# ai-forever/Kandinsky-2

Measured on AMD Instinct MI355X. Metric: UNet denoise steps/sec @ 768x768 bs=1, 50 steps, higher is better.
Workload: dtype bf16; 1 GPU; Kandinsky-2.x text2img 768x768, decoder_steps=50, bs=1/GPU (CFG batch 2x4x96x96), 2.1-architecture UNet (1.23B) p_sampler step; parity pinned against the reference's modules; head=2.1, tile_configs_measured_in_this_process=0, images_per_gpu=1, parallelism=prompt-sharded x1, weights by one RCCL broadcast, world_size_observed=1, graph=True, chains=1, loop_graph=a 5-step loop replayed as ONE hipGraph (83 replay(s) = 415 timed steps)

## Files before the change

### kandinsky-2_amd/csrc/sampler.hip

```cpp
#include <string>

#include "kernels.h"
#include "elementwise.h"

__device__ __forceinline__ const float* step_row(const SamplerParams& p) {
  const int st = p.step ? *p.step : p.step_host;
  return p.table + (int64_t)st * 8;
}

__device__ __forceinline__ float guided_eps(const SamplerParams& p, int n, int c, int pix) {
  const int64_t hw = p.HW;
  if (!p.use_cfg) return p.model_out[((int64_t)n * 8 + c) * hw + pix];
  const int bs = p.N / 2, i = n % bs;
  const float ce = p.model_out[((int64_t)i * 8 + c) * hw + pix];
  const float ue = p.model_out[((int64_t)(i + bs) * 8 + c) * hw + pix];
  return ue + p.guidance * (ce - ue);
}

__global__ __launch_bounds__(256) void sampler_x0_kernel(SamplerParams p) {
  const float* tr = step_row(p);
  const float sr = tr[0], srm1 = tr[1];
  const int64_t total = (int64_t)p.N * 4 * p.HW;
  for (int64_t i = (int64_t)blockIdx.x * 256 + threadIdx.x; i < total; i += (int64_t)gridDim.x * 256) {
    const int pix = (int)(i % p.HW);
    const int c = (int)((i / p.HW) % 4), n = (int)(i / (4 * (int64_t)p.HW));
    const float eps = guided_eps(p, n, c, pix);
    float x0 = __fsub_rn(__fmul_rn(sr, p.x[i]), __fmul_rn(srm1, eps));
    x0 = fminf(fmaxf(x0, p.clamp_lo), p.clamp_hi);
    if (p.mask != nullptr) {
      const float mk = p.mask[(int64_t)n * p.HW + pix];
      x0 = __fadd_rn(__fmul_rn(x0, 1.f - mk), __fmul_rn(p.init_img[i], mk));
    }
    p.x0_buf[i] = x0;
  }
}

__device__ __forceinline__ void hist_add_aggregated(int* hist, bool valid, uint32_t bin) {
  uint64_t todo = __ballot(valid);
  const int lane = threadIdx.x & 63;
  for (int round = 0; round < 4 && todo; ++round) {
    const int leader = __ffsll((unsigned long long)todo) - 1;
    const uint32_t lb = (uint32_t)__builtin_amdgcn_readlane((int)bin, leader);
    const uint64_t same = __ballot(valid && bin == lb) & todo;
    if (lane == leader) atomicAdd(&hist[lb], __popcll(same));
    todo &= ~same;
  }
  if ((todo >> lane) & 1) atomicAdd(&hist[bin], 1);
}

constexpr int K22_RS_BINS = 2048;
template <int KPT>
__device__ __forceinline__ uint32_t radix_select(const float* v, const uint32_t* keys, int n, int k, int* hist, uint32_t* bc, uint32_t floor_key = 0u) {
  const int tid = threadIdx.x;
  uint32_t prefix = 0, mask = 0;
#pragma unroll 1
  for (int pass = 0; pass < 3; ++pass) {
    const int shift = pass == 0 ? 21 : (pass == 1 ? 10 : 0);
    const int nb = pass == 2 ? 1024 : 2048;
    const uint32_t dmask = (uint32_t)(nb - 1);
    for (int i = tid; i < K22_RS_BINS; i += blockDim.x) hist[i] = 0;
    __syncthreads();
    if constexpr (KPT > 0) {
#pragma unroll
      for (int j = 0; j < KPT; ++j) {
        const uint32_t key = keys[j];
        const bool valid = key != 0xffffffffu && (key & mask) == prefix && key >= floor_key;
        hist_add_aggregated(hist, valid, (key >> shift) & dmask);
      }
    } else {
      for (int i0 = 0; i0 < n; i0 += blockDim.x) {
        const int i = i0 + tid;
        uint32_t key = 0;
        bool valid = false;
        if (i < n) {
          key = __float_as_uint(fabsf(v[i]));
          valid = (key & mask) == prefix;
        }
        hist_add_aggregated(hist, valid, (key >> shift) & dmask);
      }
    }
    __syncthreads();
    if (tid < 64) {
      const int per = nb >> 6;
      int run = 0;
      for (int j = 0; j < per; ++j) run += hist[tid * per + j];
      int incl = run;
#pragma unroll
      for (int o = 1; o < 64; o <<= 1) {
        const int t = __shfl_up(incl, o, 64);
        if (tid >= o) incl += t;
      }
      const int excl = incl - run;
      if (k >= excl && k < incl) {
        int acc = excl;
        for (int j = 0; j < per; ++j) {
          const int c = hist[tid * per + j];
          if (k < acc + c) { bc[0] = (uint32_t)(tid * per + j); bc[1] = (uint32_t)(k - acc); break; }
          acc += c;
        }
      }
    }
    __syncthreads();
    prefix |= bc[0] << shift;
    mask |= dmask << shift;
    k = (int)bc[1];
    __syncthreads();
  }
  return prefix;
}

template <int KPT>
__global__ __launch_bounds__(1024) void sampler_threshold_kernel(SamplerParams p) {
  __shared__ int hist[K22_RS_BINS];
  __shared__ uint32_t bc[2];
  __shared__ unsigned int succ_cnt[2];
  const int n = 4 * p.HW;
  const int k_hi = p.n_lo + 1 < n ? p.n_lo + 1 : n - 1;
  uint32_t keys[KPT > 0 ? KPT : 1];
  if constexpr (KPT > 0) {
#pragma unroll
    for (int j = 0; j < KPT; ++j) {
      const int i = j * 1024 + (int)threadIdx.x;
      keys[j] = i < n ? __float_as_uint(fabsf(p.x0_buf[i])) : 0xffffffffu;
    }
  }
  uint32_t floor_key = 0u;
  int k_sel = p.n_lo;
  if constexpr (KPT >= 16) {
    __shared__ unsigned int n_ge;
    uint32_t skey = 0xffffffffu;
    const int js = (int)threadIdx.x % KPT;
#pragma unroll
    for (int j = 0; j < KPT; ++j) skey = (j == js) ? keys[j] : skey;
    unsigned int ns_local = skey != 0xffffffffu ? 1u : 0u;
    if (threadIdx.x == 0) n_ge = 0u;
    __syncthreads();
    if (ns_local) atomicAdd(&n_ge, 1u);
    __syncthreads();
    const int ns = (int)n_ge;
    __syncthreads();
    if (ns >= 512) {
      const uint32_t pivot = radix_select<1>(nullptr, &skey, ns, (int)(ns * 0.973f), hist, bc);
      if (threadIdx.x == 0) n_ge = 0u;
      __syncthreads();
      unsigned int c = 0;
#pragma unroll
      for (int j = 0; j < KPT; ++j) c += (keys[j] != 0xffffffffu && keys[j] >= pivot) ? 1u : 0u;
#pragma unroll
      for (int o = 32; o > 0; o >>= 1) c += __shfl_xor(c, o, 64);
      if ((threadIdx.x & 63) == 0) atomicAdd(&n_ge, c);
      __syncthreads();
      const int below = n - (int)n_ge;
      if (p.n_lo >= below) { floor_key = pivot; k_sel = p.n_lo - below; }
      __syncthreads();
    }
  }
  const uint32_t ka = radix_select<KPT>(p.x0_buf, keys, n, k_sel, hist, bc, floor_key);
  if (threadIdx.x == 0) { succ_cnt[0] = 0u; succ_cnt[1] = 0xffffffffu; }
  __syncthreads();
  unsigned int cnt = 0, mn = 0xffffffffu;
  if constexpr (KPT > 0) {
#pragma unroll
    for (int j = 0; j < KPT; ++j) {
      const uint32_t key = keys[j];
      if (key == 0xffffffffu) continue;
      if (key <= ka) ++cnt;
      else mn = key < mn ? key : mn;
    }
  } else {
    for (int i = threadIdx.x; i < n; i += blockDim.x) {
      const uint32_t key = __float_as_uint(fabsf(p.x0_buf[i]));
      if (key <= ka) ++cnt;
      else mn = key < mn ? key : mn;
    }
  }
#pragma unroll
  for (int o = 32; o > 0; o >>= 1) {
    cnt += __shfl_xor(cnt, o, 64);
    const unsigned int t = __shfl_xor(mn, o, 64);
    mn = t < mn ? t : mn;
  }
  if ((threadIdx.x & 63) == 0) { atomicAdd(&succ_cnt[0], cnt); atomicMin(&succ_cnt[1], mn); }
  __syncthreads();
  if (threadIdx.x == 0) {
    const uint32_t kb = ((int)succ_cnt[0] > k_hi || k_hi == p.n_lo) ? ka : succ_cnt[1];
    const float a = __uint_as_float(ka), b = __uint_as_float(kb);
    const float t = (float)p.gamma;
    const float d = __fsub_rn(b, a);
    float r = __fadd_rn(a, __fmul_rn(d, t));
    if (t >= 0.5f) r = __fsub_rn(b, __fmul_rn(d, __fsub_rn(1.f, t)));
    p.s_buf[0] = r > 1.f ? r : 1.f;
  }
}

__global__ __launch_bounds__(256) void sampler_final_kernel(SamplerParams p) {
  const float* tr = step_row(p);
  const float c1 = tr[2], c2 = tr[3], min_log = tr[4], max_log = tr[5], nonzero = tr[6];
  const float s = (p.n_lo >= 0) ? p.s_buf[0] : 0.f;
  const int64_t total = (int64_t)p.N * 4 * p.HW;
  for (int64_t i = (int64_t)blockIdx.x * 256 + threadIdx.x; i < total; i += (int64_t)gridDim.x * 256) {
    const int pix = (int)(i % p.HW);
    const int c = (int)((i / p.HW) % 4), n = (int)(i / (4 * (int64_t)p.HW));
    float x0 = p.x0_buf[i];
    if (p.n_lo >= 0) x0 = fminf(fmaxf(x0, -s), s) / s;
    const float mean = __fadd_rn(__fmul_rn(c1, x0), __fmul_rn(c2, p.x[i]));
    const float v = p.model_out[((int64_t)n * 8 + 4 + c) * p.HW + pix];
    const float frac = (v + 1.f) / 2.f;
    const float logvar = __fadd_rn(__fmul_rn(frac, max_log), __fmul_rn(1.f - frac, min_log));
    p.x_out[i] = mean + nonzero * expf(0.5f * logvar) * p.noise[i];
    if (p.x0_out != nullptr) p.x0_out[i] = x0;
  }
}

__global__ __launch_bounds__(256) void ddim_step_kernel(const float* x, const float* model_out, const float* noise, const float* tab,
                                                        float guidance, int use_cfg, float* x_out, float* x0_out, int N, int HW) {
  const float a_t = tab[0], a_prev = tab[1], sigma = tab[2], s1m = tab[3];
  const float sq_at = sqrtf(a_t), sq_ap = sqrtf(a_prev);
  const float dirc = sqrtf(__fsub_rn(__fsub_rn(1.0f, a_prev), __fmul_rn(sigma, sigma)));
  const int64_t total = (int64_t)N * 4 * HW;
  for (int64_t i = (int64_t)blockIdx.x * 256 + threadIdx.x; i < total; i += (int64_t)gridDim.x * 256) {
    const int pix = (int)(i % HW);
    const int c = (int)((i / HW) % 4), n = (int)(i / (4 * (int64_t)HW));
    float e;
    if (use_cfg) {
      const int bs = N / 2, j = n % bs;
      const float ce = model_out[((int64_t)j * 8 + c) * HW + pix], ue = model_out[((int64_t)(j + bs) * 8 + c) * HW + pix];
      e = ue + guidance * (ce - ue);
    } else {
      e = model_out[((int64_t)n * 8 + c) * HW + pix];
    }
    const float x0 = __fdiv_rn(__fsub_rn(x[i], __fmul_rn(s1m, e)), sq_at);
    float xp = __fadd_rn(__fmul_rn(sq_ap, x0), __fmul_rn(dirc, e));
    if (noise != nullptr) xp = __fadd_rn(xp, __fmul_rn(sigma, noise[i]));
    x_out[i] = xp;
    if (x0_out != nullptr) x0_out[i] = x0;
  }
}

__global__ __launch_bounds__(256) void plms_step_kernel(const float* x, const float* model_out, const float* h1, const float* h2, const float* h3,
                                                        int order, const float* tab, float guidance, int use_cfg, float* x_out, float* e_store,
                                                        float* x0_out, int N, int HW) {
  const float a_t = tab[0], a_prev = tab[1], s1m = tab[3];
  const float sq_at = sqrtf(a_t), sq_ap = sqrtf(a_prev);
  const float dirc = sqrtf(__fsub_rn(__fsub_rn(1.0f, a_prev), 0.0f));
  const int64_t total = (int64_t)N * 4 * HW;
  for (int64_t i = (int64_t)blockIdx.x * 256 + threadIdx.x; i < total; i += (int64_t)gridDim.x * 256) {
    const int pix = (int)(i % HW);
    const int c = (int)((i / HW) % 4), n = (int)(i / (4 * (int64_t)HW));
    float e;
    if (use_cfg) {
      const int bs = N / 2, j = n % bs;
      const float ce = model_out[((int64_t)j * 8 + c) * HW + pix], ue = model_out[((int64_t)(j + bs) * 8 + c) * HW + pix];
      e = __fadd_rn(ue, __fmul_rn(guidance, __fsub_rn(ce, ue)));
    } else {
      e = model_out[((int64_t)n * 8 + c) * HW + pix];
    }
    float ep = e;
    if (order == 4) ep = __fdiv_rn(__fadd_rn(h1[i], e), 2.0f);
    else if (order == 1) ep = __fdiv_rn(__fsub_rn(__fmul_rn(3.0f, e), h1[i]), 2.0f);
    else if (order == 2) ep = __fdiv_rn(__fadd_rn(__fsub_rn(__fmul_rn(23.0f, e), __fmul_rn(16.0f, h1[i])), __fmul_rn(5.0f, h2[i])), 12.0f);
    else if (order == 3)
      ep = __fdiv_rn(__fsub_rn(__fadd_rn(__fsub_rn(__fmul_rn(55.0f, e), __fmul_rn(59.0f, h1[i])), __fmul_rn(37.0f, h2[i])), __fmul_rn(9.0f, h3[i])), 24.0f);
    const float x0 = __fdiv_rn(__fsub_rn(x[i], __fmul_rn(s1m, ep)), sq_at);
    x_out[i] = __fadd_rn(__fmul_rn(sq_ap, x0), __fmul_rn(dirc, ep));
    if (e_store != nullptr) e_store[i] = e;
    if (x0_out != nullptr) x0_out[i] = x0;
  }
}

int launch_plms_step(const float* x, const float* model_out, const float* h1, const float* h2, const float* h3, int order, const float* tab,
                     float guidance, int use_cfg, float* x_out, float* e_store, float* x0_out, int N, int HW, hipStream_t s) {
  if (N <= 0 || HW <= 0 || (use_cfg && (N & 1))) return k22_set_error(K22_EINVAL, "plms_step: bad batch");
  if (order < 0 || order > 4 || ((order == 1 || order == 4) && !h1) || (order == 2 && (!h1 || !h2)) || (order == 3 && (!h1 || !h2 || !h3)))
    return k22_set_error(K22_EINVAL, "plms_step: order 0-4 with the eps history it needs");
  const int64_t total = (int64_t)N * 4 * HW;
  int nb = (int)((total + 255) / 256);
  if (nb > 2048) nb = 2048;
  hipLaunchKernelGGL(plms_step_kernel, dim3(nb), dim3(256), 0, s, x, model_out, h1, h2, h3, order, tab, guidance, use_cfg, x_out, e_store, x0_out, N, HW);
  K22_CHECK_LAUNCH();
  return K22_OK;
}

template <bool CLIP>
__global__ __launch_bounds__(256) void dpmpp_step_kernel(const float* x, const float* model_out, const float* x0_prev, const float* tab,
                                                         float guidance, int use_cfg, float clamp_lo, float clamp_hi, float* x_out, float* x0_out,
                                                         int N, int HW) {
#pragma clang fp contract(off)
  const float a_s = tab[0], s_s = tab[1], c_x = tab[2], c_0 = tab[3];
  const float c_1 = x0_prev != nullptr ? tab[4] : 0.0f;
  const int64_t total = (int64_t)N * 4 * HW;
  for (int64_t i = (int64_t)blockIdx.x * 256 + threadIdx.x; i < total; i += (int64_t)gridDim.x * 256) {
    const int pix = (int)(i % HW);
    const int c = (int)((i / HW) % 4), n = (int)(i / (4 * (int64_t)HW));
    float e;
    if (use_cfg) {
      const int bs = N / 2, j = n % bs;
      const float ce = model_out[((int64_t)j * 8 + c) * HW + pix], ue = model_out[((int64_t)(j + bs) * 8 + c) * HW + pix];
      const float d = ce - ue;
      const float gd = guidance * d;
      e = ue + gd;
    } else {
      e = model_out[((int64_t)n * 8 + c) * HW + pix];
    }
    const float xi = x[i];
    const float se = s_s * e;
    const float num = xi - se;
    float x0 = num / a_s;
    if (CLIP) {
      if (x0 < clamp_lo) x0 = clamp_lo;
      if (x0 > clamp_hi) x0 = clamp_hi;
    }
    const float t_x = c_x * xi, t_0 = c_0 * x0;
    float out = t_x + t_0;
    if (x0_prev != nullptr) {
      const float t_1 = c_1 * x0_prev[i];
      out = out + t_1;
    }
    x_out[i] = out;
    x0_out[i] = x0;
  }
}

static int dpmpp_step_launch(const char* who, const float* x, const float* model_out, const float* x0_prev, const float* tab, float guidance,
                             int use_cfg, const float* clamp, float* x_out, float* x0_out, int N, int HW, hipStream_t s) {
  auto refuse = [who](const char* what) { return k22_set_error(K22_EINVAL, (std::string(who) + ": " + what).c_str()); };
  if (!x || !model_out || !tab || !x_out || !x0_out) return refuse("null argument");
  if (N <= 0 || HW <= 0 || (use_cfg && (N & 1))) return refuse("bad batch");
  if (x_out == x || x0_out == x || x0_out == x_out || (x0_prev && (x0_prev == x0_out || x0_prev == x_out)))
    return refuse("out of place only (x, x_out, x0_out and x0_prev are four buffers)");
  if (clamp && !(clamp[0] <= clamp[1])) return refuse("clamp_lo <= clamp_hi, neither a NaN");
  const int64_t total = (int64_t)N * 4 * HW;
  int nb = (int)((total + 255) / 256);
  if (nb > 2048) nb = 2048;
  if (clamp)
    hipLaunchKernelGGL(dpmpp_step_kernel<true>, dim3(nb), dim3(256), 0, s, x, model_out, x0_prev, tab, guidance, use_cfg, clamp[0], clamp[1], x_out,
                       x0_out, N, HW);
  else
    hipLaunchKernelGGL(dpmpp_step_kernel<false>, dim3(nb), dim3(256), 0, s, x, model_out, x0_prev, tab, guidance, use_cfg, 0.0f, 0.0f, x_out, x0_out,
                       N, HW);
  K22_CHECK_LAUNCH();
  return K22_OK;
}

int launch_dpmpp_step(const float* x, const float* model_out, const float* x0_prev, const float* tab, float guidance, int use_cfg,
                      float* x_out, float* x0_out, int N, int HW, hipStream_t s) {
  return dpmpp_step_launch("dpmpp_step", x, model_out, x0_prev, tab, guidance, use_cfg, nullptr, x_out, x0_out, N, HW, s);
}

int launch_dpmpp_step_clip(const float* x, const float* model_out, const float* x0_prev, const float* tab, float guidance, int use_cfg,
                           float clamp_lo, float clamp_hi, float* x_out, float* x0_out, int N, int HW, hipStream_t s) {
  const float clamp[2] = {clamp_lo, clamp_hi};
  return dpmpp_step_launch("dpmpp_step_clip", x, model_out, x0_prev, tab, guidance, use_cfg, clamp, x_out, x0_out, N, HW, s);
}

__global__ __launch_bounds__(256) void prepare_mask_kernel(const float* old_mask, float* out, int C, int H, int W) {
  const int i = blockIdx.x * 256 + threadIdx.x;
  if (i >= H * W) return;
  const int y = i / W, x = i - y * W;
  const int sy[6] = {y + 1, y, y + 1, y - 1, y, y - 1};
  const int sx[6] = {x, x + 1, x + 1, x, x - 1, x - 1};
  bool kill = false;
#pragma unroll
  for (int k = 0; k < 6; ++k)
    if (sy[k] >= 0 && sy[k] < H && sx[k] >= 0 && sx[k] < W && old_mask[sy[k] * W + sx[k]] != 1.0f) kill = true;
  for (int c = 0; c < C; ++c) out[(c * H + y) * W + x] = kill ? 0.0f : old_mask[(c * H + y) * W + x];
}

int launch_prepare_mask(const float* old_mask, float* out, int C, int H, int W, hipStream_t s) {
  if (C < 1 || H < 1 || W < 1 || old_mask == out) return k22_set_error(K22_EINVAL, "prepare_mask: bad arguments (out of place only)");
  hipLaunchKernelGGL(prepare_mask_kernel, dim3((H * W + 255) / 256), dim3(256), 0, s, old_mask, out, C, H, W);
  K22_CHECK_LAUNCH();
  return K22_OK;
}

int launch_ddim_step(const float* x, const float* model_out, const float* noise, const float* tab, float guidance, int use_cfg,
                     float* x_out, float* x0_out, int N, int HW, hipStream_t s) {
  if (N <= 0 || HW <= 0 || (use_cfg && (N & 1))) return k22_set_error(K22_EINVAL, "ddim_step: bad batch");
  const int64_t total = (int64_t)N * 4 * HW;
  int nb = (int)((total + 255) / 256);
  if (nb > 2048) nb = 2048;
  hipLaunchKernelGGL(ddim_step_kernel, dim3(nb), dim3(256), 0, s, x, model_out, noise, tab, guidance, use_cfg, x_out, x0_out, N, HW);
  K22_CHECK_LAUNCH();
  return K22_OK;
}

__global__ void step_advance_kernel(int* step, int delta) { *step += delta; }

int launch_sampler_step(const SamplerParams& p, hipStream_t s) {
  if (p.N <= 0 || p.HW <= 0) return k22_set_error(K22_EINVAL, "sampler: empty batch");
  if (p.use_cfg && (p.N & 1)) return k22_set_error(K22_EINVAL, "sampler: CFG needs an even batch [cond | uncond]");
  if ((p.mask == nullptr) != (p.init_img == nullptr)) return k22_set_error(K22_EINVAL, "sampler: init_img and mask go together");
  const int64_t total = (int64_t)p.N * 4 * p.HW;
  int nb = (int)((total + 255) / 256);
  if (nb > 2048) nb = 2048;
  hipLaunchKernelGGL(sampler_x0_kernel, dim3(nb), dim3(256), 0, s, p);
  K22_CHECK_LAUNCH();
  if (p.n_lo >= 0) {
    const int kpt = (4 * p.HW + 1023) / 1024;
    if (kpt <= 4) hipLaunchKernelGGL(sampler_threshold_kernel<4>, dim3(1), dim3(1024), 0, s, p);
    else if (kpt <= 16) hipLaunchKernelGGL(sampler_threshold_kernel<16>, dim3(1), dim3(1024), 0, s, p);
    else if (kpt <= 36) hipLaunchKernelGGL(sampler_threshold_kernel<36>, dim3(1), dim3(1024), 0, s, p);
    else if (kpt <= 64) hipLaunchKernelGGL(sampler_threshold_kernel<64>, dim3(1), dim3(1024), 0, s, p);
    else hipLaunchKernelGGL(sampler_threshold_kernel<0>, dim3(1), dim3(1024), 0, s, p);
    K22_CHECK_LAUNCH();
  }
  hipLaunchKernelGGL(sampler_final_kernel, dim3(nb), dim3(256), 0, s, p);
  K22_CHECK_LAUNCH();
  return K22_OK;
}

int launch_step_advance(int* step, int delta, hipStream_t s) {
  hipLaunchKernelGGL(step_advance_kernel, dim3(1), dim3(1), 0, s, step, delta);
  K22_CHECK_LAUNCH();
  return K22_OK;
}
```

Measured before the change: 148.1 steps/s.

## Replace radix select in threshold kernel with bitonic sort of pivot-filtered candidates

The dynamic-threshold quantile kernel now sorts a 1024-sample subset with a register/LDS bitonic network to pick a pivot. It compacts keys above the pivot into shared memory and sorts that small candidate set directly to read both order statistics, skipping the multi-pass radix select and the successor-count pass. The radix path stays as a fallback when the candidate count exceeds the LDS cap or the target falls below the pivot. Loads are also made branch-free through index clamping. The change adds a large amount of shared memory and many barriers in one single-block kernel, which may lower occupancy or add latency.

```diff
diff --git a/kandinsky-2_amd/csrc/sampler.hip b/kandinsky-2_amd/csrc/sampler.hip
--- a/kandinsky-2_amd/csrc/sampler.hip
+++ b/kandinsky-2_amd/csrc/sampler.hip
@@ -109,6 +109,48 @@
   return prefix;
 }
 
+constexpr int K22_RANK_CAP = 4096;
+__device__ __forceinline__ uint32_t sort_1024(uint32_t key, uint32_t (*xch)[1024]) {
+  const int tid = (int)threadIdx.x;
+  int buf = 0;
+#pragma unroll
+  for (int k = 2; k <= 1024; k <<= 1) {
+#pragma unroll
+    for (int j = k >> 1; j > 0; j >>= 1) {
+      uint32_t other;
+      if (j < 64) {
+        other = (uint32_t)__shfl_xor((int)key, j, 64);
+      } else {
+        xch[buf][tid] = key;
+        __syncthreads();
+        other = xch[buf][tid ^ j];
+        buf ^= 1;
+      }
+      const bool keep_min = ((tid & j) == 0) == ((tid & k) == 0);
+      const uint32_t lo = key < other ? key : other, hi = key < other ? other : key;
+      key = keep_min ? lo : hi;
+    }
+  }
+  return key;
+}
+
+__device__ __forceinline__ void lds_sort(uint32_t* c, int N) {
+  const int half = N >> 1;
+#pragma unroll 1
+  for (int k = 2; k <= N; k <<= 1) {
+#pragma unroll 1
+    for (int j = k >> 1; j > 0; j >>= 1) {
+      for (int t = (int)threadIdx.x; t < half; t += 1024) {
+        const int i = ((t & ~(j - 1)) << 1) | (t & (j - 1));
+        const int l = i | j;
+        const uint32_t a = c[i], b = c[l];
+        if ((a > b) == ((i & k) == 0)) { c[i] = b; c[l] = a; }
+      }
+      __syncthreads();
+    }
+  }
+}
+
 template <int KPT>
 __global__ __launch_bounds__(1024) void sampler_threshold_kernel(SamplerParams p) {
   __shared__ int hist[K22_RS_BINS];
@@ -116,79 +158,137 @@
   __shared__ unsigned int succ_cnt[2];
   const int n = 4 * p.HW;
   const int k_hi = p.n_lo + 1 < n ? p.n_lo + 1 : n - 1;
+  uint32_t skey = 0xffffffffu;
+  if constexpr (KPT >= 16) {
+    const unsigned is = (threadIdx.x % KPT) * 1024u + threadIdx.x;
+    const uint32_t v = __float_as_uint(fabsf(p.x0_buf[is < (unsigned)n ? is : (unsigned)n - 1u]));
+    skey = is < (unsigned)n ? v : 0xffffffffu;
+  }
   uint32_t keys[KPT > 0 ? KPT : 1];
   if constexpr (KPT > 0) {
 #pragma unroll
     for (int j = 0; j < KPT; ++j) {
-      const int i = j * 1024 + (int)threadIdx.x;
-      keys[j] = i < n ? __float_as_uint(fabsf(p.x0_buf[i])) : 0xffffffffu;
-    }
+      const unsigned i = j * 1024u + threadIdx.x;
+      keys[j] = __float_as_uint(fabsf(p.x0_buf[i < (unsigned)n ? i : (unsigned)n - 1u]));
+    }
+#pragma unroll
+    for (int j = 0; j < KPT; ++j) keys[j] = (int)threadIdx.x < n - j * 1024 ? keys[j] : 0xffffffffu;
   }
   uint32_t floor_key = 0u;
   int k_sel = p.n_lo;
+  uint32_t ka = 0u, kb = 0u;
+  bool ranked = false;
   if constexpr (KPT >= 16) {
-    __shared__ unsigned int n_ge;
-    uint32_t skey = 0xffffffffu;
-    const int js = (int)threadIdx.x % KPT;
-#pragma unroll
-    for (int j = 0; j < KPT; ++j) skey = (j == js) ? keys[j] : skey;
-    unsigned int ns_local = skey != 0xffffffffu ? 1u : 0u;
-    if (threadIdx.x == 0) n_ge = 0u;
-    __syncthreads();
-    if (ns_local) atomicAdd(&n_ge, 1u);
-    __syncthreads();
-    const int ns = (int)n_ge;
-    __syncthreads();
+    __shared__ uint32_t cand[K22_RANK_CAP];
+    __shared__ uint32_t xch[2][1024];
+    __shared__ unsigned int cnt[3];
+    __shared__ uint32_t pick[3];
+    const int lane = (int)threadIdx.x & 63;
+    if (threadIdx.x == 0) { cnt[0] = 0u; cnt[1] = 0u; cnt[2] = 0u; }
+    __syncthreads();
+    const uint64_t vs = __ballot(skey != 0xffffffffu);
+    if (lane == 0) atomicAdd(&cnt[0], (unsigned int)__popcll(vs));
+    __syncthreads();
+    const int ns = (int)cnt[0];
     if (ns >= 512) {
-      const uint32_t pivot = radix_select<1>(nullptr, &skey, ns, (int)(ns * 0.973f), hist, bc);
-      if (threadIdx.x == 0) n_ge = 0u;
+      const uint32_t srt = sort_1024(skey, xch);
+      if ((int)threadIdx.x == (int)(ns * 0.973f)) pick[0] = srt;
       __syncthreads();
-      unsigned int c = 0;
-#pragma unroll
-      for (int j = 0; j < KPT; ++j) c += (keys[j] != 0xffffffffu && keys[j] >= pivot) ? 1u : 0u;
-#pragma unroll
-      for (int o = 32; o > 0; o >>= 1) c += __shfl_xor(c, o, 64);
-      if ((threadIdx.x & 63) == 0) atomicAdd(&n_ge, c);
+      const uint32_t pivot = pick[0];
+      int c = 0, cge = 0;
+#pragma unroll
+      for (int j = 0; j < KPT; ++j) {
+        c += (keys[j] != 0xffffffffu && keys[j] > pivot) ? 1 : 0;
+        cge += (keys[j] != 0xffffffffu && keys[j] >= pivot) ? 1 : 0;
+      }
+      int incl = c;
+#pragma unroll
+      for (int o = 1; o < 64; o <<= 1) {
+        const int t = __shfl_up(incl, o, 64);
+        if (lane >= o) incl += t;
+      }
+#pragma unroll
+      for (int o = 32; o > 0; o >>= 1) cge += __shfl_xor(cge, o, 64);
+      int base = 0;
+      if (lane == 63) { base = (int)atomicAdd(&cnt[1], (unsigned int)incl); atomicAdd(&cnt[2], (unsigned int)cge); }
+      int pos = __shfl(base, 63, 64) + incl - c;
+#pragma unroll
+      for (int j = 0; j < KPT; ++j)
+        if (keys[j] != 0xffffffffu && keys[j] > pivot) {
+          if (pos < K22_RANK_CAP) cand[pos] = keys[j];
+          ++pos;
+        }
       __syncthreads();
-      const int below = n - (int)n_ge;
-      if (p.n_lo >= below) { floor_key = pivot; k_sel = p.n_lo - below; }
-      __syncthreads();
-    }
-  }
-  const uint32_t ka = radix_select<KPT>(p.x0_buf, keys, n, k_sel, hist, bc, floor_key);
-  if (threadIdx.x == 0) { succ_cnt[0] = 0u; succ_cnt[1] = 0xffffffffu; }
-  __syncthreads();
-  unsigned int cnt = 0, mn = 0xffffffffu;
-  if constexpr (KPT > 0) {
-#pragma unroll
-    for (int j = 0; j < KPT; ++j) {
-      const uint32_t key = keys[j];
-      if (key == 0xffffffffu) continue;
-      if (key <= ka) ++cnt;
-      else mn = key < mn ? key : mn;
-    }
-  } else {
-    for (int i = threadIdx.x; i < n; i += blockDim.x) {
-      const uint32_t key = __float_as_uint(fabsf(p.x0_buf[i]));
-      if (key <= ka) ++cnt;
-      else mn = key < mn ? key : mn;
-    }
-  }
-#pragma unroll
-  for (int o = 32; o > 0; o >>= 1) {
-    cnt += __shfl_xor(cnt, o, 64);
-    const unsigned int t = __shfl_xor(mn, o, 64);
-    mn = t < mn ? t : mn;
-  }
-  if ((threadIdx.x & 63) == 0) { atomicAdd(&succ_cnt[0], cnt); atomicMin(&succ_cnt[1], mn); }
-  __syncthreads();
+      const int m = (int)cnt[1], n_ge = (int)cnt[2];
+      const int n_eq = n_ge - m;
+      const int below = n - n_ge;
+      if (p.n_lo >= below) {
+        floor_key = pivot; k_sel = p.n_lo - below;
+        const int r0 = k_sel - n_eq, r1 = k_sel + (k_hi - p.n_lo) - n_eq;
+        if (r1 < 0) {
+          ka = pivot; kb = pivot;
+          ranked = true;
+        } else if (m <= 1024) {
+          const uint32_t s2 = sort_1024((int)threadIdx.x < m ? cand[threadIdx.x] : 0xffffffffu, xch);
+          if ((int)threadIdx.x == r0) pick[1] = s2;
+          if ((int)threadIdx.x == r1) pick[2] = s2;
+          __syncthreads();
+          ka = r0 < 0 ? pivot : pick[1]; kb = pick[2];
+          ranked = true;
+        } else if (m <= K22_RANK_CAP) {
+          int N = 2048;
+          while (N < m) N <<= 1;
+          for (int i = m + (int)threadIdx.x; i < N; i += 1024) cand[i] = 0xffffffffu;
+          __syncthreads();
+          lds_sort(cand, N);
+          ka = r0 < 0 ? pivot : cand[r0]; kb = cand[r1];
+          ranked = true;
+        }
+      }
+    }
+  }
+  if (!ranked) {
+    ka = radix_select<KPT>(p.x0_buf, keys, n, k_sel, hist, bc, floor_key);
+    if (threadIdx.x == 0) { succ_cnt[0] = 0u; succ_cnt[1] = 0xffffffffu; }
+    __syncthreads();
+    unsigned int cnt = 0, mn = 0xffffffffu;
+    if constexpr (KPT > 0) {
+#pragma unroll
+      for (int j = 0; j < KPT; ++j) {
+        const uint32_t key = keys[j];
+        if (key == 0xffffffffu) continue;
+        if (key <= ka) ++cnt;
+        else mn = key < mn ? key : mn;
+      }
+    } else {
+      for (int i = threadIdx.x; i < n; i += blockDim.x) {
+        const uint32_t key = __float_as_uint(fabsf(p.x0_buf[i]));
+        if (key <= ka) ++cnt;
+        else mn = key < mn ? key : mn;
+      }
+    }
+#pragma unroll
+    for (int o = 32; o > 0; o >>= 1) {
+      cnt += __shfl_xor(cnt, o, 64);
+      const unsigned int t = __shfl_xor(mn, o, 64);
+      mn = t < mn ? t : mn;
+    }
+    if ((threadIdx.x & 63) == 0) { atomicAdd(&succ_cnt[0], cnt); atomicMin(&succ_cnt[1], mn); }
+    __syncthreads();
+    kb = ((int)succ_cnt[0] > k_hi || k_hi == p.n_lo) ? ka : succ_cnt[1];
+  }
   if (threadIdx.x == 0) {
-    const uint32_t kb = ((int)succ_cnt[0] > k_hi || k_hi == p.n_lo) ? ka : succ_cnt[1];
+#pragma clang fp contract(off)
     const float a = __uint_as_float(ka), b = __uint_as_float(kb);
     const float t = (float)p.gamma;
-    const float d = __fsub_rn(b, a);
-    float r = __fadd_rn(a, __fmul_rn(d, t));
-    if (t >= 0.5f) r = __fsub_rn(b, __fmul_rn(d, __fsub_rn(1.f, t)));
+    const float d = b - a;
+    const float dt = d * t;
+    float r = a + dt;
+    if (t >= 0.5f) {
+      const float u = 1.f - t;
+      const float du = d * u;
+      r = b - du;
+    }
     p.s_buf[0] = r > 1.f ? r : 1.f;
   }
 }
```

New measurement: 149.1 steps/s, median of 6. About the same (+0.7%).
